# tahmidawal/Superresolution_for_PDEs

Hardware: AMD Instinct MI355X
Metric: 20->40 SR training samples/sec at batch 1024 per GPU (fwd+MSE bwd+clip+AdamW) (higher is better)
Workload: dtype f32 (h3: fp32 products from power-of-two-scaled 2-piece fp16 splits on fp16 MFMA, fp32 accumulate); 1 GPU; UNet 20->40 train step, fp32, batch 1024/GPU, 40x40; global_batch=1024, per_gpu_batch=1024, hw=40x40, parallelism=dp1

## Files before the change

superresolution_for_pdes_amd/csrc/pointwise.hip:

```cpp
#include "bn_reduce.h"

namespace srpde {

__global__ void nchw_to_nhwc_kernel(const float* __restrict__ x, float* __restrict__ out, int N, int Cin, int HW,
                                    int Cpad) {
  const long long total = (long long)N * HW;
  for (long long e = blockIdx.x * (long long)blockDim.x + threadIdx.x; e < total;
       e += (long long)gridDim.x * blockDim.x) {
    const long long n = e / HW;
    const int p = (int)(e - n * HW);
    float* o = out + e * Cpad;
    for (int c = 0; c < Cpad; ++c) o[c] = c < Cin ? x[(n * Cin + c) * HW + p] : 0.f;
  }
}

__global__ void nhwc_to_nchw_kernel(const float* __restrict__ x, int ldx, float* __restrict__ out, int N, int C,
                                    int HW) {
  const long long total = (long long)N * C * HW;
  for (long long e = blockIdx.x * (long long)blockDim.x + threadIdx.x; e < total;
       e += (long long)gridDim.x * blockDim.x) {
    const long long nc = e / HW;
    const int p = (int)(e - nc * HW);
    const long long n = nc / C;
    const int c = (int)(nc - n * C);
// ... 496 lines not shown
                                                              const float* __restrict__ b1,
                                                              const float* __restrict__ w2,
                                                              const float* __restrict__ b2, float* __restrict__ m,
                                                              float* __restrict__ h, float* __restrict__ ca) {
  extern __shared__ float sh[];
  const int n = blockIdx.x, C4 = C >> 2;
  const int c4 = threadIdx.x % C4, r0 = threadIdx.x / C4, rs = blockDim.x / C4;
  const int active = C4 * rs;
  float4 s = zero4();
  if ((int)threadIdx.x < active) {
    const float* base = x + (long long)n * HW * ldx + c4 * 4;
    for (int p = r0; p < HW; p += rs) {
      const float4 v = ld4(base + (long long)p * ldx);
      s = add4(s, v);
    }
  }
  float4* red = reinterpret_cast<float4*>(sh);
  red[threadIdx.x] = s;
  __syncthreads();
  float* ms = sh + 4 * 256;
  float* hs = ms + C;
  if ((int)threadIdx.x < C4) {
    const float4 t = rowsum4(red, C4, rs, threadIdx.x);
    const float inv = 1.f / (float)HW;
    const int c = threadIdx.x * 4;
    ms[c] = t.x * inv; ms[c + 1] = t.y * inv; ms[c + 2] = t.z * inv; ms[c + 3] = t.w * inv;
  }
  __syncthreads();
  for (int j = threadIdx.x; j < C; j += blockDim.x) m[(long long)n * C + j] = ms[j];
  for (int r = threadIdx.x; r < Cr; r += blockDim.x) {
    float a = b1[r];
    for (int c = 0; c < C; ++c) a += w1[r * C + c] * ms[c];
    a = fmaxf(a, 0.f);
    hs[r] = a;
    h[(long long)n * Cr + r] = a;
  }
  __syncthreads();
  for (int c = threadIdx.x; c < C; c += blockDim.x) {
    float a = b2[c];
    for (int r = 0; r < Cr; ++r) a += w2[c * Cr + r] * hs[r];
    ca[(long long)n * C + c] = 1.f / (1.f + expf(-a));
  }
}

__global__ __launch_bounds__(256) void att_spatial_fwd_kernel(const float* __restrict__ g, int ldg, long long P,
                                                              int G, const float* __restrict__ wg,
                                                              const float* __restrict__ bg, float* __restrict__ sa) {
  const int sub = threadIdx.x & 7;
  for (long long p = (blockIdx.x * (long long)blockDim.x + threadIdx.x) >> 3; p < P;
       p += ((long long)gridDim.x * blockDim.x) >> 3) {
    float acc = 0.f;
    const float* row = g + p * ldg;
    for (int c = sub * 4; c < G; c += 32) {
      const float4 v = ld4(row + c);
      const float4 w = ld4(wg + c);
      acc += dot4(v, w);
    }
    acc += __shfl_xor(acc, 1, 64);
    acc += __shfl_xor(acc, 2, 64);
    acc += __shfl_xor(acc, 4, 64);
    if (sub == 0) sa[p] = 1.f / (1.f + expf(-(acc + bg[0])));
  }
}

__global__ void att_apply_kernel(const float* __restrict__ x, int ldx, const float* __restrict__ ca,
                                 const float* __restrict__ sa, float* __restrict__ out, int ldo, long long P, int HW,
                                 int C) {
  const int C4 = C >> 2;
  const long long total = P * C4;
  for (long long e = blockIdx.x * (long long)blockDim.x + threadIdx.x; e < total;
       e += (long long)gridDim.x * blockDim.x) {
    const long long p = e / C4;
    const int c = (int)(e - p * C4) * 4;
    const long long n = p / HW;
    const float4 v = ld4(x + p * ldx + c);
    const float4 a = ld4(ca + n * C + c);
    const float s = sa[p];
    float4 o;
    o.x = (v.x * a.x) * s; o.y = (v.y * a.y) * s; o.z = (v.z * a.z) * s; o.w = (v.w * a.w) * s;
    *reinterpret_cast<float4*>(out + p * ldo + c) = o;
  }
}

__global__ __launch_bounds__(256) void att_bwd_pixel_kernel(const float* __restrict__ dout, int lddo,
                                                            const float* __restrict__ x, int ldx,
                                                            const float* __restrict__ ca,
                                                            const float* __restrict__ sa, long long P, int HW, int C,
                                                            float* __restrict__ dsa_pre) {
  const int sub = threadIdx.x & 7;
  for (long long p = (blockIdx.x * (long long)blockDim.x + threadIdx.x) >> 3; p < P;
       p += ((long long)gridDim.x * blockDim.x) >> 3) {
    const long long n = p / HW;
    float acc = 0.f;
    for (int c = sub * 4; c < C; c += 32) {
      const float4 d = ld4(dout + p * lddo + c);
      const float4 v = ld4(x + p * ldx + c);
      const float4 a = ld4(ca + n * C + c);
      acc += d.x * (v.x * a.x) + d.y * (v.y * a.y) + d.z * (v.z * a.z) + d.w * (v.w * a.w);
    }
    acc += __shfl_xor(acc, 1, 64);
    acc += __shfl_xor(acc, 2, 64);
    acc += __shfl_xor(acc, 4, 64);
    if (sub == 0) {
      const float s = sa[p];
      dsa_pre[p] = acc * (1.f - s) * s;
    }
  }
}

__global__ __launch_bounds__(256) void att_bwd_channel_kernel(
    const float* __restrict__ dout, int lddo, const float* __restrict__ x, int ldx, const float* __restrict__ sa,
    int HW, int C, int Cr, const float* __restrict__ w1, const float* __restrict__ w2, const float* __restrict__ m,
    const float* __restrict__ h, const float* __restrict__ ca, float* __restrict__ dm,
    float* __restrict__ dw1_rows, float* __restrict__ db1_rows, float* __restrict__ dw2_rows,
    float* __restrict__ db2_rows) {
  extern __shared__ float sh[];
  const int n = blockIdx.x, C4 = C >> 2;
  const int c4 = threadIdx.x % C4, r0 = threadIdx.x / C4, rs = blockDim.x / C4;
  const int active = C4 * rs;
  float4 s = zero4();
  if ((int)threadIdx.x < active) {
    const long long pb = (long long)n * HW;
    for (int p = r0; p < HW; p += rs) {
      const float4 d = ld4(dout + (pb + p) * lddo + c4 * 4);
      const float4 v = ld4(x + (pb + p) * ldx + c4 * 4);
      const float q = sa[pb + p];
      s.x += (d.x * q) * v.x; s.y += (d.y * q) * v.y; s.z += (d.z * q) * v.z; s.w += (d.w * q) * v.w;
    }
  }
  float4* red = reinterpret_cast<float4*>(sh);
  red[threadIdx.x] = s;
  __syncthreads();
  float* dpre = sh + 4 * 256;
  float* dh = dpre + C;
  if ((int)threadIdx.x < C4) {
    const float4 t = rowsum4(red, C4, rs, threadIdx.x);
    const int c = threadIdx.x * 4;
    const float tv[4] = {t.x, t.y, t.z, t.w};
#pragma unroll
    for (int k = 0; k < 4; ++k) {
      const float a = ca[(long long)n * C + c + k];
      dpre[c + k] = tv[k] * (1.f - a) * a;
    }
  }
  __syncthreads();
  for (int c = threadIdx.x; c < C; c += blockDim.x) db2_rows[(long long)n * C + c] = dpre[c];
  for (int r = threadIdx.x; r < Cr; r += blockDim.x) {
    float a = 0.f;
    for (int c = 0; c < C; ++c) a += w2[c * Cr + r] * dpre[c];
    a = h[(long long)n * Cr + r] > 0.f ? a : 0.f;
    dh[r] = a;
    db1_rows[(long long)n * Cr + r] = a;
  }
  __syncthreads();
  for (int c = threadIdx.x; c < C; c += blockDim.x) {
    float a = 0.f;
    for (int r = 0; r < Cr; ++r) a += w1[r * C + c] * dh[r];
    dm[(long long)n * C + c] = a / (float)HW;
  }
}

__global__ __launch_bounds__(256) void att_bwd_sample_kernel(
    const float* __restrict__ dout, int lddo, const float* __restrict__ x, int ldx, const float* __restrict__ sa,
    int HW, int C, int Cr, const float* __restrict__ w1, const float* __restrict__ w2, const float* __restrict__ m,
    const float* __restrict__ h, const float* __restrict__ ca, float* __restrict__ dm, float* __restrict__ dw1_rows,
    float* __restrict__ db1_rows, float* __restrict__ dw2_rows, float* __restrict__ db2_rows,
    float* __restrict__ dsa_pre) {
  extern __shared__ float sh[];
  const int n = blockIdx.x, C4 = C >> 2;
  const int c4 = threadIdx.x % C4, r0 = threadIdx.x / C4, rs = blockDim.x / C4;
  float4 s = zero4();
  {
    const float4 a = ld4(ca + (long long)n * C + c4 * 4);
    const long long pb = (long long)n * HW;
    for (int p = r0; p < HW; p += rs) {
      const float4 d = ld4(dout + (pb + p) * lddo + c4 * 4);
      const float4 v = ld4(x + (pb + p) * ldx + c4 * 4);
      const float q = sa[pb + p];
      s.x += (d.x * q) * v.x; s.y += (d.y * q) * v.y; s.z += (d.z * q) * v.z; s.w += (d.w * q) * v.w;
      float dot = d.x * (v.x * a.x) + d.y * (v.y * a.y) + d.z * (v.z * a.z) + d.w * (v.w * a.w);
      for (int o = C4 >> 1; o > 0; o >>= 1) dot += __shfl_xor(dot, o, 64);
      if (c4 == 0) dsa_pre[pb + p] = dot * (1.f - q) * q;
    }
  }
  float4* red = reinterpret_cast<float4*>(sh);
  red[threadIdx.x] = s;
  __syncthreads();
  float* dpre = sh + 4 * 256;
  float* dh = dpre + C;
  if ((int)threadIdx.x < C4) {
    const float4 t = rowsum4(red, C4, rs, threadIdx.x);
    const int c = threadIdx.x * 4;
    const float tv[4] = {t.x, t.y, t.z, t.w};
#pragma unroll
    for (int k = 0; k < 4; ++k) {
      const float a = ca[(long long)n * C + c + k];
      dpre[c + k] = tv[k] * (1.f - a) * a;
    }
  }
  __syncthreads();
  for (int c = threadIdx.x; c < C; c += blockDim.x) db2_rows[(long long)n * C + c] = dpre[c];
  for (int r = threadIdx.x; r < Cr; r += blockDim.x) {
    float a = 0.f;
    for (int c = 0; c < C; ++c) a += w2[c * Cr + r] * dpre[c];
    a = h[(long long)n * Cr + r] > 0.f ? a : 0.f;
    dh[r] = a;
    db1_rows[(long long)n * Cr + r] = a;
  }
  __syncthreads();
  for (int c = threadIdx.x; c < C; c += blockDim.x) {
    float a = 0.f;
    for (int r = 0; r < Cr; ++r) a += w1[r * C + c] * dh[r];
    dm[(long long)n * C + c] = a / (float)HW;
  }
}

__global__ void att_bwd_dx_kernel(const float* __restrict__ dout, int lddo, const float* __restrict__ ca,
                                  const float* __restrict__ sa, const float* __restrict__ dm, float* __restrict__ dx,
                                  int lddx, long long P, int HW, int C, int accumulate) {
  const int C4 = C >> 2;
  const long long total = P * C4;
  for (long long e = blockIdx.x * (long long)blockDim.x + threadIdx.x; e < total;
       e += (long long)gridDim.x * blockDim.x) {
    const long long p = e / C4;
    const int c = (int)(e - p * C4) * 4;
    const long long n = p / HW;
    const float4 d = ld4(dout + p * lddo + c);
    const float4 a = ld4(ca + n * C + c);
    const float4 g = ld4(dm + n * C + c);
    const float s = sa[p];
    float4 o = gate_dx4(d, s, a, g);
    float* dst = dx + p * lddx + c;
    if (accumulate) o = add4(o, ld4(dst));
    st4(dst, o);
  }
}

__global__ void att_bwd_gating_kernel(const float* __restrict__ dsa_pre, const float* __restrict__ wg,
                                      float* __restrict__ dg, int lddg, long long P, int G, int accumulate) {
  const int G4 = G >> 2;
  const long long total = P * G4;
  for (long long e = blockIdx.x * (long long)blockDim.x + threadIdx.x; e < total;
       e += (long long)gridDim.x * blockDim.x) {
    const long long p = e / G4;
    const int c = (int)(e - p * G4) * 4;
    const float s = dsa_pre[p];
    const float4 w = ld4(wg + c);
    float4 o = scale4(s, w);
    float* dst = dg + p * lddg + c;
    if (accumulate) o = add4(o, ld4(dst));
    st4(dst, o);
  }
}

__global__ __launch_bounds__(256) void weighted_colsum_kernel(const float* __restrict__ v, int ldv,
                                                              const float* __restrict__ s, long long P, int C,
                                                              int rows_per_blk, float2* __restrict__ part) {
  extern __shared__ float4 red4[];
  const int C4 = C >> 2;
  const int c4 = threadIdx.x % C4, r0 = threadIdx.x / C4, rs = blockDim.x / C4;
  const int active = C4 * rs;
  float4 acc = zero4();
  float sacc = 0.f;
  const long long pb = (long long)blockIdx.x * rows_per_blk;
  const long long pe = min(P, pb + rows_per_blk);
  if ((int)threadIdx.x < active) {
    auto row = [&](const float4& a, float w) {
      acc.x += a.x * w; acc.y += a.y * w; acc.z += a.z * w; acc.w += a.w * w;
      if (c4 == 0) sacc += w;
    };
    long long p = pb + r0;
    for (; p + 3 * rs < pe; p += 4 * rs) {
      float4 a[4];
      float w[4];
#pragma unroll
      for (int u = 0; u < 4; ++u) {
        a[u] = ld4(v + (p + u * rs) * ldv + c4 * 4);
        w[u] = s[p + u * rs];
      }
#pragma unroll
      for (int u = 0; u < 4; ++u) row(a[u], w[u]);
    }
    for (; p < pe; p += rs) row(ld4(v + p * ldv + c4 * 4), s[p]);
  }
  red4[threadIdx.x] = acc;
  red4[256 + threadIdx.x] = make_float4(sacc, 0.f, 0.f, 0.f);
  __syncthreads();
  if ((int)threadIdx.x < C4) {
    float4 t = zero4();
    float ts = 0.f;
    for (int r = 0; r < rs; ++r) {
      const float4 a = red4[r * C4 + threadIdx.x];
      t.x += a.x; t.y += a.y; t.z += a.z; t.w += a.w;
      if (threadIdx.x == 0) ts += red4[256 + r * C4].x;
    }
    float2* o = part + (size_t)blockIdx.x * (C + 1);
    const int c = threadIdx.x * 4;
    o[c] = make_float2(t.x, 0.f); o[c + 1] = make_float2(t.y, 0.f);
    o[c + 2] = make_float2(t.z, 0.f); o[c + 3] = make_float2(t.w, 0.f);
    if (threadIdx.x == 0) o[C] = make_float2(ts, 0.f);
  }
}

__global__ __launch_bounds__(1024) void outer_sum_kernel(const float* __restrict__ a, int la,
                                                         const float* __restrict__ b, int lb, int n,
                                                         float* __restrict__ out) {
  __shared__ double red[16][64];
  const int i = blockIdx.x, jl = threadIdx.x & 63, grp = threadIdx.x >> 6;
  const int j = blockIdx.y * 64 + jl;
  double s = 0.0;
  if (j < lb) {
    int k = grp;
    for (; k + 7 * 16 < n; k += 8 * 16) {
      float av[8], bv[8];
#pragma unroll
      for (int u = 0; u < 8; ++u) {
        av[u] = a ? a[(long long)(k + 16 * u) * la + i] : 1.f;
        bv[u] = b ? b[(long long)(k + 16 * u) * lb + j] : 1.f;
      }
#pragma unroll
      for (int u = 0; u < 8; ++u) s += (double)av[u] * (double)bv[u];
    }
    for (; k < n; k += 16) {
      const double av = a ? (double)a[(long long)k * la + i] : 1.0;
      const double bv = b ? (double)b[(long long)k * lb + j] : 1.0;
      s += av * bv;
    }
  }
  red[grp][jl] = s;
  __syncthreads();
  if (grp == 0 && j < lb) {
    double t = 0.0;
    for (int g = 0; g < 16; ++g) t += red[g][jl];
    out[(long long)i * lb + j] = (float)t;
  }
}

__global__ void rowsum_kernel(const float* __restrict__ rows, int n, int len, float* __restrict__ out, int stride_in,
                              int accumulate) {
  const int j = blockIdx.x * blockDim.x + threadIdx.x;
  if (j >= len) return;
  double s = 0.0;
  for (int k = 0; k < n; ++k) s += rows[(long long)k * stride_in + j];
  out[j] = accumulate ? out[j] + (float)s : (float)s;
}

__global__ void partsum_kernel(const float2* __restrict__ part, int nblk, int len, float* __restrict__ out) {
  const int j = blockIdx.x;
  __shared__ double a[256];
  double s = 0.0;
  for (int k = threadIdx.x; k < nblk; k += 256) s += part[(size_t)k * len + j].x;
  a[threadIdx.x] = s;
  __syncthreads();
  for (int t = 128; t > 0; t >>= 1) {
    if ((int)threadIdx.x < t) a[threadIdx.x] += a[threadIdx.x + t];
    __syncthreads();
  }
  if (threadIdx.x == 0) out[j] = (float)a[0];
}

__global__ void head_fwd_kernel(const float* __restrict__ z, int ldz, int C, const float* __restrict__ wf,
                                const float* __restrict__ bf, const float* __restrict__ xin, int xin_c, int HW,
                                long long P, float* __restrict__ out) {
  for (long long p = blockIdx.x * (long long)blockDim.x + threadIdx.x; p < P; p += (long long)gridDim.x * blockDim.x) {
    float acc = 0.f;
    for (int c = 0; c < C; c += 4) {
      const float4 v = ld4(z + p * ldz + c);
      acc += v.x * wf[c] + v.y * wf[c + 1] + v.z * wf[c + 2] + v.w * wf[c + 3];
    }
    const long long n = p / HW;
    const int q = (int)(p - n * HW);
    out[p] = (acc + bf[0]) + xin[(n * xin_c) * HW + q];
  }
}

__global__ void head_bwd_dz_kernel(const float* __restrict__ dout, const float* __restrict__ wf, int C,
                                   float* __restrict__ dz, int lddz, long long P) {
  const int C4 = C >> 2;
  const long long total = P * C4;
  for (long long e = blockIdx.x * (long long)blockDim.x + threadIdx.x; e < total;
       e += (long long)gridDim.x * blockDim.x) {
    const long long p = e / C4;
    const int c = (int)(e - p * C4) * 4;
    const float d = dout[p];
    *reinterpret_cast<float4*>(dz + p * lddz + c) = make_float4(d * wf[c], d * wf[c + 1], d * wf[c + 2], d * wf[c + 3]);
  }
}

__global__ __launch_bounds__(256) void mse_partial_kernel(const float* __restrict__ y, const float* __restrict__ t,
                                                          long long n, double* __restrict__ part) {
  __shared__ double red[256];
  double s = 0.0;
  for (long long i = blockIdx.x * (long long)blockDim.x + threadIdx.x; i < n; i += (long long)gridDim.x * blockDim.x) {
    const float d = y[i] - t[i];
    s += (double)(d * d);
  }
  red[threadIdx.x] = s;
  __syncthreads();
  for (int k = 128; k > 0; k >>= 1) {
    if ((int)threadIdx.x < k) red[threadIdx.x] += red[threadIdx.x + k];
    __syncthreads();
  }
  if (threadIdx.x == 0) part[blockIdx.x] = red[0];
}

__global__ void mse_final_kernel(const double* __restrict__ part, int nblk, long long n, float* __restrict__ loss) {
  __shared__ double red[256];
  double s = 0.0;
  for (int k = threadIdx.x; k < nblk; k += 256) s += part[k];
  red[threadIdx.x] = s;
  __syncthreads();
  for (int k = 128; k > 0; k >>= 1) {
    if ((int)threadIdx.x < k) red[threadIdx.x] += red[threadIdx.x + k];
    __syncthreads();
  }
  if (threadIdx.x == 0) loss[0] = (float)(red[0] / (double)n);
}

__global__ void mse_bwd_kernel(const float* __restrict__ y, const float* __restrict__ t, long long n,
                               const float* __restrict__ gout, float* __restrict__ dy) {
  const float g = gout ? gout[0] : 1.f;
  const float norm = 2.f / (float)n;
  for (long long i = blockIdx.x * (long long)blockDim.x + threadIdx.x; i < n; i += (long long)gridDim.x * blockDim.x)
    dy[i] = norm * (y[i] - t[i]) * g;
}

static bool colsum_ok(int C) { return C % 4 == 0 && C >= 4 && C <= 1024; }
static bool att_bwd_counts_ok(int c, int gc) { return c % 32 == 0 && c >= 32 && c <= 1024 && colsum_ok(gc); }

static int colsum_blocks(long long P, int C, int* rpb) {
  const int rs = 256 / (C >> 2);
  long long r = (P + 1023) / 1024;
  r = (r + rs - 1) / rs * rs;
  if (r < rs) r = rs;
  *rpb = (int)r;
  return (int)((P + r - 1) / r);
}

}

using namespace srpde;

extern "C" {

int srpde_nchw_to_nhwc(const float* x, float* out, int n, int cin, int h, int w, int cpad, hipStream_t stream) {
  SRPDE_CHECK_ARG(x && out && cpad >= cin, "srpde_nchw_to_nhwc: bad args");
  hipLaunchKernelGGL(nchw_to_nhwc_kernel, dim3(grid_for((long long)n * h * w)), dim3(256), 0, stream, x, out, n, cin,
                     h * w, cpad);
  SRPDE_LAUNCH_CHECK("srpde_nchw_to_nhwc");
  return 0;
}

int srpde_nhwc_to_nchw(const float* x, int ldx, float* out, int n, int c, int h, int w, hipStream_t stream) {
  SRPDE_CHECK_ARG(x && out && n > 0 && c > 0 && ldx >= c, "srpde_nhwc_to_nchw: bad args");
  hipLaunchKernelGGL(nhwc_to_nchw_kernel, dim3(grid_for((long long)n * c * h * w)), dim3(256), 0, stream, x, ldx, out,
                     n, c, h * w);
  SRPDE_LAUNCH_CHECK("srpde_nhwc_to_nchw");
  return 0;
}

int srpde_axpy_channel(float* y, const float* x, int n, int c, int hw, int ch, float alpha, hipStream_t stream) {
  SRPDE_CHECK_ARG(y && x && n > 0 && ch >= 0 && ch < c && hw > 0, "srpde_axpy_channel: bad args");
  hipLaunchKernelGGL(axpy_channel_kernel, dim3(grid_for((long long)n * hw)), dim3(256), 0, stream, y, x, n, c, hw, ch,
                     alpha);
  SRPDE_LAUNCH_CHECK("srpde_axpy_channel");
  return 0;
}

int srpde_maxpool2x2_fwd(const float* x, int ldx, float* out, int ldo, int n, int h, int w, int c,
                         hipStream_t stream) {
  SRPDE_CHECK_ARG(x && out && c % 4 == 0 && h % 2 == 0 && w % 2 == 0, "srpde_maxpool2x2_fwd: bad args");
  launch_px_or_grid_stride(
      (long long)n * (h / 2) * (w / 2), c,
      [&](dim3 g, dim3 b, unsigned npix) {
        hipLaunchKernelGGL(maxpool2_fwd_px_kernel, g, b, 0, stream, x, ldx, out, ldo, npix, h, w);
      },
      [&](dim3 g) { hipLaunchKernelGGL(maxpool2_fwd_kernel, g, dim3(256), 0, stream, x, ldx, out, ldo, n, h, w, c); });
  SRPDE_LAUNCH_CHECK("srpde_maxpool2x2_fwd");
  return 0;
}

int srpde_maxpool2x2_bwd(const float* x, int ldx, const float* dout, int lddo, float* dx, int lddx, int n, int h,
                         int w, int c, int accumulate, hipStream_t stream) {
  SRPDE_CHECK_ARG(x && dout && dx && c % 4 == 0 && h % 2 == 0 && w % 2 == 0, "srpde_maxpool2x2_bwd: bad args");
  launch_px_or_grid_stride(
      (long long)n * (h / 2) * (w / 2), c,
      [&](dim3 g, dim3 b, unsigned npix) {
        hipLaunchKernelGGL(maxpool2_bwd_px_kernel, g, b, 0, stream, x, ldx, dout, lddo, dx, lddx, npix, h, w, accumulate);
      },
      [&](dim3 g) {
        hipLaunchKernelGGL(maxpool2_bwd_kernel, g, dim3(256), 0, stream, x, ldx, dout, lddo, dx, lddx, n, h, w, c,
                           accumulate);
      });
  SRPDE_LAUNCH_CHECK("srpde_maxpool2x2_bwd");
  return 0;
}

int srpde_pde_dataset_assemble(const float* u_coarse, const float* u_fine, const float* theta_fine,
                               const float* f_fine, const float* stats, int theta_constant, int n, int hc, int wc,
                               int hf, int wf, float* inputs, float* targets, hipStream_t stream) {
  SRPDE_CHECK_ARG(u_coarse && u_fine && theta_fine && f_fine && stats && inputs && targets,
                  "srpde_pde_dataset_assemble: null");
  SRPDE_CHECK_ARG(n >= 0 && hc >= 1 && wc >= 1 && hf >= hc && wf >= wc, "srpde_pde_dataset_assemble: bad shape");
  if (n == 0) return 0;
  hipLaunchKernelGGL(pde_dataset_kernel, dim3(grid_for((long long)n * hf * wf)), dim3(256), 0, stream, u_coarse,
                     u_fine, theta_fine, f_fine, stats, theta_constant, n, hc, wc, hf, wf, inputs, targets);
  SRPDE_LAUNCH_CHECK("srpde_pde_dataset_assemble");
  return 0;
}

int srpde_upsample_bilinear_fwd(const float* x, int ldx, float* out, int ldo, int n, int h, int w, int ho, int wo,
                                int c, hipStream_t stream) {
  SRPDE_CHECK_ARG(x && out && c > 0, "srpde_upsample_bilinear_fwd: bad args");
  if (c % 4 != 0 || ldx % 4 != 0 || ldo % 4 != 0) {
    hipLaunchKernelGGL(upsample_fwd_scalar_kernel, dim3(grid_for((long long)n * ho * wo * c)), dim3(256), 0, stream,
                       x, ldx, out, ldo, n, h, w, ho, wo, c);
    SRPDE_LAUNCH_CHECK("srpde_upsample_bilinear_fwd");
    return 0;
  }
  launch_px_or_grid_stride(
      (long long)n * ho * wo, c,
      [&](dim3 g, dim3 b, unsigned npix) {
        hipLaunchKernelGGL(upsample_fwd_px_kernel, g, b, 0, stream, x, ldx, out, ldo, npix, h, w, ho, wo);
      },
      [&](dim3 g) {
        hipLaunchKernelGGL(upsample_fwd_kernel, g, dim3(256), 0, stream, x, ldx, out, ldo, n, h, w, ho, wo, c);
      });
  SRPDE_LAUNCH_CHECK("srpde_upsample_bilinear_fwd");
  return 0;
}

int srpde_upsample_bilinear_gate_fwd(const float* x, int ldx, float* out, int ldo, int n, int h, int w, int ho,
                                      int wo, int c, const float* wg, const float* bg, float* sa, hipStream_t stream) {
  SRPDE_CHECK_ARG(x && out && wg && bg && sa && ldx % 4 == 0 && ldo % 4 == 0 && c % 4 == 0 && c / 4 >= 1 &&
                      c / 4 <= 64 && ((c / 4) & (c / 4 - 1)) == 0,
                  "srpde_upsample_bilinear_gate_fwd: bad args (c / 4 a power of two <= 64)");
  dim3 g, b;
  SRPDE_CHECK_ARG(px_geometry((long long)n * ho * wo, c, &g, &b), "srpde_upsample_bilinear_gate_fwd: bad geometry");
  g.x = (g.x + UPX - 1) / UPX;
  hipLaunchKernelGGL(upsample_gate_fwd_px_kernel, g, b, 0, stream, x, ldx, out, ldo, (unsigned)(n * ho * wo), h, w,
                     ho, wo, wg, bg, sa);
  SRPDE_LAUNCH_CHECK("srpde_upsample_bilinear_gate_fwd");
  return 0;
}

size_t srpde_upsample_gate_sa_workspace_size(int n, int h, int w) { return (size_t)n * h * w * sizeof(float); }

int srpde_upsample_gate_sa(const float* x, int ldx, int n, int h, int w, int ho, int wo, int c, const float* wg,
                           const float* bg, float* sa, void* workspace, size_t ws_bytes, hipStream_t stream) {
  SRPDE_CHECK_ARG(x && wg && bg && sa && workspace && ldx % 4 == 0 && c % 4 == 0 && c / 4 >= 1 && c / 4 <= 64 &&
                      ((c / 4) & (c / 4 - 1)) == 0 && n > 0 && h > 0 && w > 0 && ho > 0 && wo > 0,
                  "srpde_upsample_gate_sa: bad args (c / 4 a power of two <= 64)");
  SRPDE_CHECK_ARG(ws_bytes >= srpde_upsample_gate_sa_workspace_size(n, h, w), "srpde_upsample_gate_sa: workspace");
  float* t = static_cast<float*>(workspace);
  dim3 g, b;
  SRPDE_CHECK_ARG(px_geometry((long long)n * h * w, c, &g, &b), "srpde_upsample_gate_sa: bad geometry");
  hipLaunchKernelGGL(gate_dot_px_kernel, g, b, 0, stream, x, ldx, (unsigned)(n * h * w), wg, t);
  SRPDE_LAUNCH_CHECK("srpde_upsample_gate_sa(dot)");
  const unsigned np = (unsigned)(n * ho * wo);
  hipLaunchKernelGGL(up_sigmoid_kernel, dim3((np + 255) / 256), dim3(256), 0, stream, t, sa, np, h, w, ho, wo, bg);
  SRPDE_LAUNCH_CHECK("srpde_upsample_gate_sa(up)");
  return 0;
}

static size_t att_lds_bytes(int c) { return (4 * 256 + c + c / 8) * sizeof(float); }

static void launch_att_channel(const float* x, int ldx, int n, int hw, int c, const float* w1, const float* b1,
                               const float* w2, const float* b2, float* m, float* hbuf, float* ca, hipStream_t stream) {
  hipLaunchKernelGGL(att_channel_fwd_kernel, dim3(n), dim3(256), att_lds_bytes(c), stream, x, ldx, hw, c, c / 8, w1, b1,
                     w2, b2, m, hbuf, ca);
}
static void launch_att_spatial(const float* g, int ldg, long long P, int gc, const float* wg, const float* bg, float* sa,
                               hipStream_t stream) {
  hipLaunchKernelGGL(att_spatial_fwd_kernel, dim3(grid_for(P * 8)), dim3(256), 0, stream, g, ldg, P, gc, wg, bg, sa);
}
static void launch_att_apply(const float* x, int ldx, const float* ca, const float* sa, float* out, int ldo, long long P,
                             int hw, int c, hipStream_t stream) {
  hipLaunchKernelGGL(att_apply_kernel, dim3(grid_for(P * (c / 4))), dim3(256), 0, stream, x, ldx, ca, sa, out, ldo, P,
                     hw, c);
}

int srpde_att_apply_fwd(const float* x, int ldx, int n, int hw, int c, const float* ca, const float* sa, float* out,
                        int ldo, hipStream_t stream) {
  SRPDE_CHECK_ARG(x && ca && sa && out && c % 4 == 0, "srpde_att_apply_fwd: bad args");
  launch_att_apply(x, ldx, ca, sa, out, ldo, (long long)n * hw, hw, c, stream);
  SRPDE_LAUNCH_CHECK("srpde_att_apply_fwd");
  return 0;
}

int srpde_upsample_bilinear_bwd_gated(const float* dout, int lddo, const float* dsa, const float* wg, float* dx,
                                      int lddx, int n, int h, int w, int ho, int wo, int c, int accumulate,
                                      hipStream_t stream) {
  SRPDE_CHECK_ARG(dout && dsa && wg && dx && c % 4 == 0 && lddo % 4 == 0 && lddx % 4 == 0 && ho >= h && wo >= w,
                  "srpde_upsample_bilinear_bwd_gated: bad args");
  SRPDE_CHECK_ARG(upsample_gather_ok(h, ho) && upsample_gather_ok(w, wo),
                  "srpde_upsample_bilinear_bwd_gated: upsampling ratio above 4 (%dx%d -> %dx%d)", h, w, ho, wo);
  if (upsample_rows_ok(h, w, ho, wo, c, lddo, lddx)) {
    launch_upsample_bwd_rows<true>(dout, lddo, dx, lddx, n, h, w, ho, wo, c, accumulate, dsa, wg, stream);
    SRPDE_LAUNCH_CHECK("srpde_upsample_bilinear_bwd_gated");
    return 0;
  }
  dim3 g, b;
  SRPDE_CHECK_ARG(px_geometry((long long)n * h * w, c, &g, &b),
                  "srpde_upsample_bilinear_bwd_gated: needs c / 4 a power of two <= 256 (c=%d)", c);
  hipLaunchKernelGGL(upsample_bwd_px_kernel, g, b, 0, stream, dout, lddo, dx, lddx, (unsigned)(n * h * w), h, w, ho,
                     wo, accumulate, dsa, wg);
  SRPDE_LAUNCH_CHECK("srpde_upsample_bilinear_bwd_gated");
  return 0;
}

int srpde_upsample_bwd_bn_supported(int h, int w, int ho, int wo, int c, int lddo, int lddx) {
  return upsample_gather_ok(h, ho) && upsample_gather_ok(w, wo) && upsample_rows_ok(h, w, ho, wo, c, lddo, lddx) ? 1
                                                                                                               : 0;
}

int srpde_upsample_bilinear_bwd_gated_bn(const float* dout, int lddo, const float* dsa, const float* wg, float* dx,
                                         int lddx, int n, int h, int w, int ho, int wo, int c, const float* y, int ldy,
                                         const float* mean, const float* invstd, const float* gamma,
                                         const float* beta, int flags, void* part, float* da_max,
                                         hipStream_t stream) {
  SRPDE_CHECK_ARG(dout && dsa && wg && dx && y && mean && invstd && gamma && beta && part && da_max && ldy % 4 == 0 &&
                      aligned16(y) && aligned16(dx) && aligned16(dout),
                  "srpde_upsample_bilinear_bwd_gated_bn: null argument / alignment");
  SRPDE_CHECK_ARG(ho >= h && wo >= w && srpde_upsample_bwd_bn_supported(h, w, ho, wo, c, lddo, lddx),
                  "srpde_upsample_bilinear_bwd_gated_bn: shape outside the row-blocked kernel "
                  "(srpde_upsample_bwd_bn_supported)");
  const UpBnArgs bn{y, ldy, mean, invstd, gamma, beta, flags & SRPDE_BN_RELU, static_cast<float2*>(part), da_max};
  launch_upsample_bwd_rows<true>(dout, lddo, dx, lddx, n, h, w, ho, wo, c, 0, dsa, wg, stream, &bn);
  SRPDE_LAUNCH_CHECK("srpde_upsample_bilinear_bwd_gated_bn");
  return 0;
}

int srpde_upsample_bilinear_bwd(const float* dout, int lddo, float* dx, int lddx, int n, int h, int w, int ho,
                                int wo, int c, int accumulate, hipStream_t stream) {
  SRPDE_CHECK_ARG(dout && dx && c % 4 == 0 && ho >= h && wo >= w, "srpde_upsample_bilinear_bwd: bad args");
  SRPDE_CHECK_ARG(upsample_gather_ok(h, ho) && upsample_gather_ok(w, wo),
                  "srpde_upsample_bilinear_bwd: upsampling ratio above 4 (%dx%d -> %dx%d)", h, w, ho, wo);
  if (upsample_rows_ok(h, w, ho, wo, c, lddo, lddx)) {
    launch_upsample_bwd_rows<false>(dout, lddo, dx, lddx, n, h, w, ho, wo, c, accumulate, nullptr, nullptr, stream);
    SRPDE_LAUNCH_CHECK("srpde_upsample_bilinear_bwd");
    return 0;
  }
  launch_px_or_grid_stride(
      (long long)n * h * w, c,
      [&](dim3 g, dim3 b, unsigned npix) {
        hipLaunchKernelGGL(upsample_bwd_px_kernel, g, b, 0, stream, dout, lddo, dx, lddx, npix, h, w, ho, wo, accumulate);
      },
      [&](dim3 g) {
        hipLaunchKernelGGL(upsample_bwd_kernel, g, dim3(256), 0, stream, dout, lddo, dx, lddx, n, h, w, ho, wo, c,
                           accumulate);
      });
  SRPDE_LAUNCH_CHECK("srpde_upsample_bilinear_bwd");
  return 0;
}

int srpde_att_channel_fwd(const float* x, int ldx, int n, int hw, int c, const float* w1, const float* b1,
                          const float* w2, const float* b2, float* m, float* hbuf, float* ca, hipStream_t stream) {
  SRPDE_CHECK_ARG(x && w1 && b1 && w2 && b2 && m && hbuf && ca, "srpde_att_channel_fwd: null");
  SRPDE_CHECK_ARG(c % 32 == 0 && c <= 1024, "srpde_att_channel_fwd: channel count");
  launch_att_channel(x, ldx, n, hw, c, w1, b1, w2, b2, m, hbuf, ca, stream);
  SRPDE_LAUNCH_CHECK("srpde_att_channel_fwd");
  return 0;
}

int srpde_att_gate_fwd(const float* x, int ldx, const float* g, int ldg, int n, int hw, int c, int gc,
                       const float* ca, const float* wg, const float* bg, float* sa, float* out, int ldo,
                       hipStream_t stream) {
  SRPDE_CHECK_ARG(x && g && ca && wg && bg && sa && out, "srpde_att_gate_fwd: null");
  SRPDE_CHECK_ARG(c % 32 == 0 && gc % 4 == 0 && c <= 1024, "srpde_att_gate_fwd: channel counts");
  const long long P = (long long)n * hw;
  launch_att_spatial(g, ldg, P, gc, wg, bg, sa, stream);
  SRPDE_LAUNCH_CHECK("srpde_att_gate_fwd(spatial)");
  launch_att_apply(x, ldx, ca, sa, out, ldo, P, hw, c, stream);
  SRPDE_LAUNCH_CHECK("srpde_att_gate_fwd(apply)");
  return 0;
}

int srpde_att_fwd(const float* x, int ldx, const float* g, int ldg, int n, int hw, int c, int gc, const float* w1,
                  const float* b1, const float* w2, const float* b2, const float* wg, const float* bg, float* m,
                  float* hbuf, float* ca, float* sa, float* out, int ldo, hipStream_t stream) {
  SRPDE_CHECK_ARG(x && g && w1 && b1 && w2 && b2 && wg && bg && m && hbuf && ca && sa && out,
                  "srpde_att_fwd: null");
  SRPDE_CHECK_ARG(c % 32 == 0 && gc % 4 == 0 && c <= 1024, "srpde_att_fwd: channel counts");
  launch_att_channel(x, ldx, n, hw, c, w1, b1, w2, b2, m, hbuf, ca, stream);
  SRPDE_LAUNCH_CHECK("srpde_att_fwd(channel)");
  const long long P = (long long)n * hw;
  launch_att_spatial(g, ldg, P, gc, wg, bg, sa, stream);
  SRPDE_LAUNCH_CHECK("srpde_att_fwd(spatial)");
  launch_att_apply(x, ldx, ca, sa, out, ldo, P, hw, c, stream);
  SRPDE_LAUNCH_CHECK("srpde_att_fwd(apply)");
  return 0;
}

size_t srpde_att_bwd_workspace_size(int n, int hw, int c, int gc) {
  if (!att_bwd_counts_ok(c, gc)) return 0;
  const long long P = (long long)n * hw;
  const int cr = c / 8;
  int rpb;
  const int nb = colsum_blocks(P, gc, &rpb);
  size_t f = (size_t)P
             + (size_t)n * c
             + (size_t)n * cr * c * 2
             + (size_t)n * (cr + c)
             + (size_t)nb * (gc + 1) * 2;
  return f * sizeof(float) + 256;
}

int srpde_att_bwd(const float* dout, int lddo, const float* x, int ldx, const float* g, int ldg, int n, int hw,
                  int c, int gc, const float* w1, const float* w2, const float* wg, const float* m, const float* hbuf,
                  const float* ca, const float* sa, float* dx, int lddx, int dx_accumulate, float* dg, int lddg,
                  int dg_accumulate, float* dw1, float* db1, float* dw2, float* db2, float* dwg, float* dbg,
                  void* workspace, size_t ws_bytes, hipStream_t stream) {
  SRPDE_CHECK_ARG(dout && x && g && workspace, "srpde_att_bwd: null");
  SRPDE_CHECK_ARG(att_bwd_counts_ok(c, gc), "srpde_att_bwd: channel counts (c %% 32, gc %% 4, both <= 1024)");
  if (ws_bytes < srpde_att_bwd_workspace_size(n, hw, c, gc)) {
    set_error("srpde_att_bwd: workspace too small");
    return kErrWorkspace;
  }
  const long long P = (long long)n * hw;
  const int cr = c / 8;
  float* dsa = static_cast<float*>(workspace);
  float* dm = dsa + P;
  float* dw1r = dm + (size_t)n * c;
  float* dw2r = dw1r + (size_t)n * cr * c;
  float* db1r = dw2r + (size_t)n * cr * c;
  float* db2r = db1r + (size_t)n * cr;
  float2* part = reinterpret_cast<float2*>(db2r + (size_t)n * c + 2);
  part = reinterpret_cast<float2*>((reinterpret_cast<uintptr_t>(part) + 15) & ~uintptr_t(15));

  const size_t lds = att_lds_bytes(c);
  if (c == 64 || c == 128 || c == 256) {
    hipLaunchKernelGGL(att_bwd_sample_kernel, dim3(n), dim3(256), lds, stream, dout, lddo, x, ldx, sa, hw, c, cr, w1,
                       w2, m, hbuf, ca, dm, dw1r, db1r, dw2r, db2r, dsa);
    SRPDE_LAUNCH_CHECK("srpde_att_bwd(sample)");
  } else {
    hipLaunchKernelGGL(att_bwd_pixel_kernel, dim3(grid_for(P * 8)), dim3(256), 0, stream, dout, lddo, x, ldx, ca,
                       sa, P, hw, c, dsa);
    SRPDE_LAUNCH_CHECK("srpde_att_bwd(pixel)");
    hipLaunchKernelGGL(att_bwd_channel_kernel, dim3(n), dim3(256), lds, stream, dout, lddo, x, ldx, sa, hw, c, cr,
                       w1, w2, m, hbuf, ca, dm, dw1r, db1r, dw2r, db2r);
    SRPDE_LAUNCH_CHECK("srpde_att_bwd(channel)");
  }
  if (dx != nullptr) {
    hipLaunchKernelGGL(att_bwd_dx_kernel, dim3(grid_for(P * (c / 4))), dim3(256), 0, stream, dout, lddo, ca, sa, dm,
                       dx, lddx, P, hw, c, dx_accumulate);
    SRPDE_LAUNCH_CHECK("srpde_att_bwd(dx)");
  }
  if (dg != nullptr) {
    hipLaunchKernelGGL(att_bwd_gating_kernel, dim3(grid_for(P * (gc / 4))), dim3(256), 0, stream, dsa, wg, dg, lddg,
                       P, gc, dg_accumulate);
    SRPDE_LAUNCH_CHECK("srpde_att_bwd(gating)");
  }
  if (dw1 == nullptr) return 0;
  return srpde_att_bwd_params(g, ldg, n, hw, c, gc, m, hbuf, dw1, db1, dw2, db2, dwg, dbg, workspace, ws_bytes,
                              stream);
}

__global__ __launch_bounds__(256) void upsample_t_scalar_kernel(const float* __restrict__ dsa, float* __restrict__ st,
                                                                int n, int h, int w, int ho, int wo) {
  const long long q = (long long)blockIdx.x * blockDim.x + threadIdx.x;
  if (q >= (long long)n * h * w) return;
  const int ix = (int)(q % w), iy = (int)((q / w) % h), nn = (int)(q / ((long long)w * h));
  int ylo, yhi, xlo, xhi;
  cand_range(iy, h, ho, &ylo, &yhi);
  cand_range(ix, w, wo, &xlo, &xhi);
  const float* base = dsa + (size_t)nn * ho * wo;
  float s = 0.f;
  for (int oy = ylo; oy <= yhi; ++oy) {
    bool hy;
    const float wy = cand_weight(oy, iy, h, ho, &hy);
    if (!hy) continue;
    float r = 0.f;
    for (int ox = xlo; ox <= xhi; ++ox) {
      bool hx;
      const float wx = cand_weight(ox, ix, w, wo, &hx);
      if (hx) r += wx * base[(size_t)oy * wo + ox];
    }
    s += wy * r;
  }
  st[q] = s;
}

static void att_params_outer(int n, int c, const float* m, const float* hbuf, const float* db1r, const float* db2r,
                             float* dw1, float* db1, float* dw2, float* db2, hipStream_t stream) {
  const int cr = c / 8;
  hipLaunchKernelGGL(outer_sum_kernel, dim3(cr, ceil_div(c, 64)), dim3(1024), 0, stream, db1r, cr, m, c, n, dw1);
  hipLaunchKernelGGL(outer_sum_kernel, dim3(c, ceil_div(cr, 64)), dim3(1024), 0, stream, db2r, c, hbuf, cr, n, dw2);
  hipLaunchKernelGGL(outer_sum_kernel, dim3(1, ceil_div(cr, 64)), dim3(1024), 0, stream, (const float*)nullptr, 1,
                     db1r, cr, n, db1);
  hipLaunchKernelGGL(outer_sum_kernel, dim3(1, ceil_div(c, 64)), dim3(1024), 0, stream, (const float*)nullptr, 1,
                     db2r, c, n, db2);
}

int srpde_att_bwd_params_lowres(const float* d, int ldd, int n, int h, int w, int ho, int wo, int c, int gc,
                                const float* m, const float* hbuf, float* dw1, float* db1, float* dw2, float* db2,
                                float* dwg, float* dbg, void* workspace, size_t ws_bytes, hipStream_t stream) {
  SRPDE_CHECK_ARG(d && m && hbuf && dw1 && db1 && dw2 && db2 && dwg && dbg && workspace && ldd % 4 == 0 && ho >= h &&
                      wo >= w,
                  "srpde_att_bwd_params_lowres: bad args");
  SRPDE_CHECK_ARG(att_bwd_counts_ok(c, gc),
                  "srpde_att_bwd_params_lowres: channel counts (c %% 32, gc %% 4, both <= 1024)");
  const int hw = ho * wo;
  if (ws_bytes < srpde_att_bwd_workspace_size(n, hw, c, gc)) {
    set_error("srpde_att_bwd_params_lowres: workspace too small");
    return kErrWorkspace;
  }
  const long long P = (long long)n * hw, Plo = (long long)n * h * w;
  const int cr = c / 8;
  float* dsa = static_cast<float*>(workspace);
  float* dm = dsa + P;
  float* dw1r = dm + (size_t)n * c;
  float* dw2r = dw1r + (size_t)n * cr * c;
  float* db1r = dw2r + (size_t)n * cr * c;
  float* db2r = db1r + (size_t)n * cr;
  float2* part = reinterpret_cast<float2*>(db2r + (size_t)n * c + 2);
  part = reinterpret_cast<float2*>((reinterpret_cast<uintptr_t>(part) + 15) & ~uintptr_t(15));
  SRPDE_CHECK_ARG(Plo <= 2LL * n * cr * c, "srpde_att_bwd_params_lowres: low-res field larger than its scratch");
  float* st = dw1r;
  att_params_outer(n, c, m, hbuf, db1r, db2r, dw1, db1, dw2, db2, stream);
  SRPDE_LAUNCH_CHECK("srpde_att_bwd_params_lowres(rowsum)");
  hipLaunchKernelGGL(upsample_t_scalar_kernel, dim3((unsigned)((Plo + 255) / 256)), dim3(256), 0, stream, dsa, st, n, h,
                     w, ho, wo);
  SRPDE_LAUNCH_CHECK("srpde_att_bwd_params_lowres(transpose)");
  int rpb;
  const int nb = colsum_blocks(Plo, gc, &rpb);
  hipLaunchKernelGGL(weighted_colsum_kernel, dim3(nb), dim3(256), 2 * 256 * sizeof(float4), stream, d, ldd, st, Plo,
                     gc, rpb, part);
  SRPDE_LAUNCH_CHECK("srpde_att_bwd_params_lowres(colsum)");
  hipLaunchKernelGGL(partsum_kernel, dim3(gc), dim3(256), 0, stream, part, nb, gc + 1, dwg);
  hipLaunchKernelGGL(partsum_kernel, dim3(1), dim3(256), 0, stream, part + gc, nb, gc + 1, dbg);
  SRPDE_LAUNCH_CHECK("srpde_att_bwd_params_lowres(partsum)");
  return 0;
}

int srpde_att_bwd_params(const float* g, int ldg, int n, int hw, int c, int gc, const float* m, const float* hbuf,
                         float* dw1, float* db1, float* dw2, float* db2, float* dwg, float* dbg, void* workspace,
                         size_t ws_bytes, hipStream_t stream) {
  SRPDE_CHECK_ARG(g && m && hbuf && dw1 && db1 && dw2 && db2 && dwg && dbg && workspace,
                  "srpde_att_bwd_params: null");
  SRPDE_CHECK_ARG(att_bwd_counts_ok(c, gc), "srpde_att_bwd_params: channel counts (c %% 32, gc %% 4, both <= 1024)");
  if (ws_bytes < srpde_att_bwd_workspace_size(n, hw, c, gc)) {
    set_error("srpde_att_bwd_params: workspace too small");
    return kErrWorkspace;
  }
  const long long P = (long long)n * hw;
  const int cr = c / 8;
  float* dsa = static_cast<float*>(workspace);
  float* dm = dsa + P;
  float* dw1r = dm + (size_t)n * c;
  float* dw2r = dw1r + (size_t)n * cr * c;
  float* db1r = dw2r + (size_t)n * cr * c;
  float* db2r = db1r + (size_t)n * cr;
  float2* part = reinterpret_cast<float2*>(db2r + (size_t)n * c + 2);
  part = reinterpret_cast<float2*>((reinterpret_cast<uintptr_t>(part) + 15) & ~uintptr_t(15));
  (void)dw1r; (void)dw2r; (void)cr;
  att_params_outer(n, c, m, hbuf, db1r, db2r, dw1, db1, dw2, db2, stream);
  SRPDE_LAUNCH_CHECK("srpde_att_bwd(rowsum)");
  int rpb;
  const int nb = colsum_blocks(P, gc, &rpb);
  hipLaunchKernelGGL(weighted_colsum_kernel, dim3(nb), dim3(256), 2 * 256 * sizeof(float4), stream, g, ldg, dsa, P,
                     gc, rpb, part);
  SRPDE_LAUNCH_CHECK("srpde_att_bwd(colsum)");
  hipLaunchKernelGGL(partsum_kernel, dim3(gc), dim3(256), 0, stream, part, nb, gc + 1, dwg);
  hipLaunchKernelGGL(partsum_kernel, dim3(1), dim3(256), 0, stream, part + gc, nb, gc + 1, dbg);
  SRPDE_LAUNCH_CHECK("srpde_att_bwd(partsum)");
  return 0;
}

int srpde_head_fwd(const float* z, int ldz, int c, const float* wf, const float* bf, const float* xin, int xin_c,
                   int n, int hw, float* out, hipStream_t stream) {
  SRPDE_CHECK_ARG(z && wf && bf && xin && out && c % 4 == 0, "srpde_head_fwd: bad args");
  const long long P = (long long)n * hw;
  hipLaunchKernelGGL(head_fwd_kernel, dim3(grid_for(P)), dim3(256), 0, stream, z, ldz, c, wf, bf, xin, xin_c, hw, P,
                     out);
  SRPDE_LAUNCH_CHECK("srpde_head_fwd");
  return 0;
}

size_t srpde_head_bwd_workspace_size(int n, int hw, int c) {
  if (!colsum_ok(c)) return 0;
  int rpb;
  const int nb = colsum_blocks((long long)n * hw, c, &rpb);
  return (size_t)nb * (c + 1) * sizeof(float2);
}

int srpde_head_bwd(const float* dout, const float* z, int ldz, int c, const float* wf, int n, int hw, float* dz,
                   int lddz, float* dwf, float* dbf, void* workspace, size_t ws_bytes, hipStream_t stream) {
  SRPDE_CHECK_ARG(dout && z && wf && dz && dwf && dbf && workspace, "srpde_head_bwd: bad args");
  SRPDE_CHECK_ARG(colsum_ok(c), "srpde_head_bwd: channel count (c %% 4, 4 <= c <= 1024)");
  if (ws_bytes < srpde_head_bwd_workspace_size(n, hw, c)) {
    set_error("srpde_head_bwd: workspace too small");
    return kErrWorkspace;
  }
  const long long P = (long long)n * hw;
  hipLaunchKernelGGL(head_bwd_dz_kernel, dim3(grid_for(P * (c / 4))), dim3(256), 0, stream, dout, wf, c, dz, lddz, P);
  SRPDE_LAUNCH_CHECK("srpde_head_bwd(dz)");
  int rpb;
  const int nb = colsum_blocks(P, c, &rpb);
  float2* part = static_cast<float2*>(workspace);
  hipLaunchKernelGGL(weighted_colsum_kernel, dim3(nb), dim3(256), 2 * 256 * sizeof(float4), stream, z, ldz, dout, P,
                     c, rpb, part);
  hipLaunchKernelGGL(partsum_kernel, dim3(c), dim3(256), 0, stream, part, nb, c + 1, dwf);
  hipLaunchKernelGGL(partsum_kernel, dim3(1), dim3(256), 0, stream, part + c, nb, c + 1, dbf);
  SRPDE_LAUNCH_CHECK("srpde_head_bwd(reduce)");
  return 0;
}

size_t srpde_mse_workspace_size(void) { return 1024 * sizeof(double); }

int srpde_mse_fwd(const float* y, const float* t, long long n, float* loss, void* workspace, size_t ws_bytes,
                  hipStream_t stream) {
  SRPDE_CHECK_ARG(y && t && loss && workspace && ws_bytes >= 1024 * sizeof(double), "srpde_mse_fwd: bad args");
  const int nb = (int)std::min<long long>(1024, std::max<long long>(1, (n + 255) / 256));
  hipLaunchKernelGGL(mse_partial_kernel, dim3(nb), dim3(256), 0, stream, y, t, n, static_cast<double*>(workspace));
  hipLaunchKernelGGL(mse_final_kernel, dim3(1), dim3(256), 0, stream, static_cast<const double*>(workspace), nb, n,
                     loss);
  SRPDE_LAUNCH_CHECK("srpde_mse_fwd");
  return 0;
}

int srpde_mse_bwd(const float* y, const float* t, long long n, const float* gout, float* dy, hipStream_t stream) {
  SRPDE_CHECK_ARG(y && t && dy, "srpde_mse_bwd: bad args");
  hipLaunchKernelGGL(mse_bwd_kernel, dim3(grid_for(n)), dim3(256), 0, stream, y, t, n, gout, dy);
  SRPDE_LAUNCH_CHECK("srpde_mse_bwd");
  return 0;
}

}
```

Baseline: 36740 samples/s.

## Fuse attention weight/bias outer-product reductions into one tiled LDS-staged kernel

Replaces four launches of a naive per-output outer_sum kernel with one templated kernel. Each block computes a 64 x TR tile of dw1 or dw2 by staging chunks of both operands in shared memory with software-prefetched float4 loads, and accumulates 4x4 register tiles in double precision. Bias gradients are folded into the blocks that own the first tile. This cuts redundant global reads (each input row was reloaded per output row) and launch overhead, at the cost of more register and LDS use.

```diff
diff --git a/superresolution_for_pdes_amd/csrc/pointwise.hip b/superresolution_for_pdes_amd/csrc/pointwise.hip
--- a/superresolution_for_pdes_amd/csrc/pointwise.hip
+++ b/superresolution_for_pdes_amd/csrc/pointwise.hip
@@ -822,37 +822,121 @@
   }
 }
 
-__global__ __launch_bounds__(1024) void outer_sum_kernel(const float* __restrict__ a, int la,
-                                                         const float* __restrict__ b, int lb, int n,
-                                                         float* __restrict__ out) {
-  __shared__ double red[16][64];
-  const int i = blockIdx.x, jl = threadIdx.x & 63, grp = threadIdx.x >> 6;
-  const int j = blockIdx.y * 64 + jl;
-  double s = 0.0;
-  if (j < lb) {
-    int k = grp;
-    for (; k + 7 * 16 < n; k += 8 * 16) {
-      float av[8], bv[8];
-#pragma unroll
-      for (int u = 0; u < 8; ++u) {
-        av[u] = a ? a[(long long)(k + 16 * u) * la + i] : 1.f;
-        bv[u] = b ? b[(long long)(k + 16 * u) * lb + j] : 1.f;
+template <int TR>
+__global__ __launch_bounds__(1024) void att_outer_kernel(const float* __restrict__ m, const float* __restrict__ hbuf,
+                                                         const float* __restrict__ db1r,
+                                                         const float* __restrict__ db2r, int n, int c, int cr,
+                                                         float* __restrict__ dw1, float* __restrict__ db1,
+                                                         float* __restrict__ dw2, float* __restrict__ db2) {
+  constexpr int CH = 128, D = 3, TQ = TR / 4, NQ = CH * TQ, G = 256 / TR, HC = TR / 2;
+  static_assert((TR == 8 || TR == 16 || TR == 32) && NQ <= 1024, "tile");
+  __shared__ __attribute__((aligned(16))) double sh[16 * 8 * 64];
+  double* nd = sh;
+  float* wf = reinterpret_cast<float*>(sh + CH * 32);
+  const int tid = threadIdx.x, jl = tid & 63;
+  const int l16 = tid & 15, cq = (tid >> 6) % TQ, grp = (tid >> 6) / TQ * 4 + ((tid >> 4) & 3);
+  const int jt = (c + 63) / 64, tiles = jt * ((cr + TR - 1) / TR);
+  const bool second = (int)blockIdx.x >= tiles;
+  const int tile = (int)blockIdx.x - (second ? tiles : 0);
+  const int j0 = (tile % jt) * 64, r0 = (tile / jt) * TR, j = j0 + jl;
+  const bool bias = second ? r0 == 0 : j0 == 0;
+  const float* __restrict__ W = second ? db2r : m;
+  const float* __restrict__ N = second ? hbuf : db1r;
+  const bool nquads = (reinterpret_cast<uintptr_t>(N) & 15) == 0, wquads = (reinterpret_cast<uintptr_t>(W) & 15) == 0;
+  const int ns = tid / TQ, nr = (tid % TQ) * 4, ws = tid >> 4, wj = l16 * 4;
+  const bool nload = tid < NQ && r0 + nr < cr, wload = j0 + wj < c;
+
+  auto quad = [](const float* p, bool aligned) { return aligned ? ld4(p) : make_float4(p[0], p[1], p[2], p[3]); };
+  auto fetch = [&](float4& nq, float4& wq0, float4& wq1, int k0) {
+    nq = wq0 = wq1 = zero4();
+    if (nload && k0 + ns < n) nq = quad(N + (long long)(k0 + ns) * cr + r0 + nr, nquads);
+    if (wload && k0 + ws < n) wq0 = quad(W + (long long)(k0 + ws) * c + j0 + wj, wquads);
+    if (wload && k0 + ws + 64 < n) wq1 = quad(W + (long long)(k0 + ws + 64) * c + j0 + wj, wquads);
+  };
+
+  double acc[4][4], bs[4] = {0.0, 0.0, 0.0, 0.0};
+#pragma unroll
+  for (int a = 0; a < 4; ++a)
+#pragma unroll
+    for (int b = 0; b < 4; ++b) acc[a][b] = 0.0;
+  float4 nq[D], wq0[D], wq1[D];
+#pragma unroll
+  for (int d = 0; d < D; ++d) fetch(nq[d], wq0[d], wq1[d], d * CH);
+  for (int kd = 0; kd < n; kd += D * CH) {
+#pragma unroll
+    for (int d = 0; d < D; ++d) {
+      const int k0 = kd + d * CH;
+      if (k0 >= n) break;
+      if (tid < NQ) {
+        double* p = nd + ns * TR + nr;
+        p[0] = (double)nq[d].x; p[1] = (double)nq[d].y; p[2] = (double)nq[d].z; p[3] = (double)nq[d].w;
       }
-#pragma unroll
-      for (int u = 0; u < 8; ++u) s += (double)av[u] * (double)bv[u];
-    }
-    for (; k < n; k += 16) {
-      const double av = a ? (double)a[(long long)k * la + i] : 1.0;
-      const double bv = b ? (double)b[(long long)k * lb + j] : 1.0;
-      s += av * bv;
-    }
-  }
-  red[grp][jl] = s;
-  __syncthreads();
-  if (grp == 0 && j < lb) {
-    double t = 0.0;
-    for (int g = 0; g < 16; ++g) t += red[g][jl];
-    out[(long long)i * lb + j] = (float)t;
+      st4(wf + ws * 64 + wj, wq0[d]);
+      st4(wf + (ws + 64) * 64 + wj, wq1[d]);
+      if (bias) {
+        if (second) {
+          bs[0] += (double)wq0[d].x + (double)wq1[d].x; bs[1] += (double)wq0[d].y + (double)wq1[d].y;
+          bs[2] += (double)wq0[d].z + (double)wq1[d].z; bs[3] += (double)wq0[d].w + (double)wq1[d].w;
+        } else {
+          bs[0] += (double)nq[d].x; bs[1] += (double)nq[d].y; bs[2] += (double)nq[d].z; bs[3] += (double)nq[d].w;
+        }
+      }
+      __syncthreads();
+      fetch(nq[d], wq0[d], wq1[d], k0 + D * CH);
+      const int se = min(CH, n - k0);
+#pragma unroll 2
+      for (int s = grp; s < se; s += G) {
+        const float4 w = ld4(wf + s * 64 + wj);
+        const double* np = nd + s * TR + cq * 4;
+        const double wd[4] = {(double)w.x, (double)w.y, (double)w.z, (double)w.w};
+        const double nv[4] = {np[0], np[1], np[2], np[3]};
+#pragma unroll
+        for (int a = 0; a < 4; ++a)
+#pragma unroll
+          for (int b = 0; b < 4; ++b) acc[a][b] += wd[a] * nv[b];
+      }
+      __syncthreads();
+    }
+  }
+
+#pragma unroll
+  for (int rr = 0; rr < 2; ++rr) {
+#pragma unroll
+    for (int b = 0; b < 2; ++b)
+#pragma unroll
+      for (int a = 0; a < 4; ++a) sh[((grp * HC) + cq * 2 + b) * 64 + wj + a] = acc[a][2 * rr + b];
+    __syncthreads();
+    if (tid < HC * 64) {
+      const int col = tid >> 6, r = r0 + (col >> 1) * 4 + 2 * rr + (col & 1);
+      double t = 0.0;
+      for (int g = 0; g < G; ++g) t += sh[(g * HC + col) * 64 + jl];
+      if (j < c && r < cr) {
+        if (second) dw2[(long long)j * cr + r] = (float)t;
+        else dw1[(long long)r * c + j] = (float)t;
+      }
+    }
+    __syncthreads();
+  }
+  if (bias) {
+    if (second) {
+#pragma unroll
+      for (int a = 0; a < 4; ++a) sh[ws * 64 + wj + a] = bs[a];
+    } else if (tid < NQ) {
+#pragma unroll
+      for (int b = 0; b < 4; ++b) sh[ns * TR + nr + b] = bs[b];
+    }
+    __syncthreads();
+    if (second) {
+      if (tid < 64 && j < c) {
+        double t = 0.0;
+        for (int k = 0; k < 64; ++k) t += sh[k * 64 + jl];
+        db2[j] = (float)t;
+      }
+    } else if (tid < TR && r0 + tid < cr) {
+      double t = 0.0;
+      for (int k = 0; k < CH; ++k) t += sh[k * TR + tid];
+      db1[r0 + tid] = (float)t;
+    }
   }
 }
 
@@ -1304,12 +1388,13 @@
 static void att_params_outer(int n, int c, const float* m, const float* hbuf, const float* db1r, const float* db2r,
                              float* dw1, float* db1, float* dw2, float* db2, hipStream_t stream) {
   const int cr = c / 8;
-  hipLaunchKernelGGL(outer_sum_kernel, dim3(cr, ceil_div(c, 64)), dim3(1024), 0, stream, db1r, cr, m, c, n, dw1);
-  hipLaunchKernelGGL(outer_sum_kernel, dim3(c, ceil_div(cr, 64)), dim3(1024), 0, stream, db2r, c, hbuf, cr, n, dw2);
-  hipLaunchKernelGGL(outer_sum_kernel, dim3(1, ceil_div(cr, 64)), dim3(1024), 0, stream, (const float*)nullptr, 1,
-                     db1r, cr, n, db1);
-  hipLaunchKernelGGL(outer_sum_kernel, dim3(1, ceil_div(c, 64)), dim3(1024), 0, stream, (const float*)nullptr, 1,
-                     db2r, c, n, db2);
+  auto launch = [&](auto kernel, int tr) {
+    hipLaunchKernelGGL(kernel, dim3(2 * ceil_div(c, 64) * ceil_div(cr, tr)), dim3(1024), 0, stream, m, hbuf, db1r,
+                       db2r, n, c, cr, dw1, db1, dw2, db2);
+  };
+  if (cr > 16) launch(att_outer_kernel<32>, 32);
+  else if (cr > 8) launch(att_outer_kernel<16>, 16);
+  else launch(att_outer_kernel<8>, 8);
 }
 
 int srpde_att_bwd_params_lowres(const float* d, int ldd, int n, int h, int w, int ho, int wo, int c, int gc,
```

Result: no change. 36910 samples/s (median of 6 runs) (+0.5%).
